# haesungpyun/seoul_tourism_recommendation_NGCF

Measured on NVIDIA B200. Metric: ngcf_epoch_time_fwd_bwd_bpr, lower is better.
Workload: dtype f32

## Files before the change

seoul_tourism_recommendation_ngcf_b200/csrc/dense.cu:

```cuda
#include <stdlib.h>
#include <string.h>

#include "common.cuh"

namespace {

__global__ void pack_weights_kernel(const float* __restrict__ W1, const float* __restrict__ b1,
                                    const float* __restrict__ W2, const float* __restrict__ b2, int d_in, int d_out,
                                    float* __restrict__ wcat, float* __restrict__ bias_eff) {
    const int total = 2 * d_in * d_out;
    for (int i = blockIdx.x * blockDim.x + threadIdx.x; i < total; i += gridDim.x * blockDim.x) {
        const int k = i / d_out, o = i % d_out;
        wcat[i] = k < d_in ? W1[o * d_in + k] : W2[o * d_in + (k - d_in)];
    }
    for (int o = blockIdx.x * blockDim.x + threadIdx.x; o < d_out; o += gridDim.x * blockDim.x)
        bias_eff[o] = 2.0f * b1[o] + b2[o];
}

struct PackAllArgs {
    const float* W1[NGCF_MAX_LAYERS];
    const float* b1[NGCF_MAX_LAYERS];
    const float* W2[NGCF_MAX_LAYERS];
    const float* b2[NGCF_MAX_LAYERS];
    float* wcat[NGCF_MAX_LAYERS];
// ... 492 lines not shown

extern "C" int ngcf_dense_bwd(const float* gE_next, const int32_t* slot, const float* gsum, int64_t ld_gsum,
                              int col_off, const float* E_out, const float* S, const float* E, int64_t n_rows,
                              int d_in, int d_out, const float* W1, const float* W2, float slope,
                              const float* mess_mult, const uint32_t* mess_bits, float mess_p, uint64_t seed,
                              const uint64_t* seed_dev, int layer, int64_t row_offset, int gh_normalized, float* gS,
                              float* gEl, float* gW1, float* gb1, float* gW2, float* gb2, float* gM_scratch, void* stream) {
    NGCF_REQUIRE(E_out && S && E && W1 && W2 && gS && gEl && gW1 && gb1 && gW2 && gb2, "dense_bwd: null pointer");
    NGCF_REQUIRE(!slot || gsum, "dense_bwd: slot given without gsum");
    NGCF_REQUIRE(d_in > 0 && d_in <= NGCF_MAX_WIDTH && d_out > 0 && d_out <= NGCF_MAX_WIDTH,
                 "dense_bwd: widths %d -> %d not in [1,%d]", d_in, d_out, NGCF_MAX_WIDTH);
    NGCF_REQUIRE(mess_p >= 0.f && mess_p < 1.f, "dense_bwd: mess_p %f not in [0,1)", mess_p);
    NGCF_REQUIRE(n_rows >= 0 && n_rows < ((int64_t)1 << 31), "dense_bwd: n_rows %lld", (long long)n_rows);
    if (n_rows == 0) return NGCF_OK;
    if (ngcf_use_tensor_cores() && gM_scratch && ngcf_dense_bwd_tc_eligible(d_in, d_out, gh_normalized) && aligned16(S) &&
        aligned16(E) && aligned16(gS) && aligned16(gEl) && aligned16(gM_scratch))
        return ngcf_dense_bwd_tc(gE_next, slot, gsum, ld_gsum, col_off, E_out, S, E, n_rows, d_in, d_out, W1, W2,
                                 slope, mess_mult, mess_bits, mess_p, seed, seed_dev, layer, row_offset, gh_normalized, gS,
                                 gEl, gW1, gb1, gW2, gb2, gM_scratch, as_stream(stream));
    BwdArgs a{gE_next, slot, gsum, ld_gsum, col_off, E_out, S, E, n_rows, d_in, d_out, W1, W2, slope, mess_mult,
              mess_bits, mess_p, seed, seed_dev, layer, gS, gEl, gW1, gb1, gW2, gb2, 0, row_offset, gh_normalized};
    int rc;
    if (d_in <= 64 && d_out <= 64) {
        constexpr int DC = 64, R = 64, T = 256;
        a.n_tiles = (int)ceil_div64(n_rows, R);
        const size_t smem = sizeof(float) * (2 * DC * DC + 3 * R * (DC + 4) + (T / 32) * DC);
        const int grid = (int)min((int64_t)a.n_tiles, (int64_t)ngcf_num_sms() * 2);
        if ((rc = set_smem(dense_bwd_kernel<DC, R, T>, smem)) != NGCF_OK) return rc;
        dense_bwd_kernel<DC, R, T><<<grid, T, smem, as_stream(stream)>>>(a);
    } else {
        constexpr int DC = 128, R = 32, T = 512;
// ... 45 lines not shown
```

seoul_tourism_recommendation_ngcf_b200/csrc/dense_tc.cu:

```cuda
#include <stdlib.h>
#include <string.h>

#include "tc.cuh"
#include "tmap.h"

namespace {

using namespace tc;

__device__ long long g_bwd_dbg[4][8][8];
__device__ int g_bwd_dbg_on = 0;
#define BWD_STAMP(role, it, k)                                                   \
    do {                                                                         \
        if (dbg && lane == 0 && (it) < 8) g_bwd_dbg[role][it][k] = clock64();    \
    } while (0)

constexpr int TC_ROWS = 128;
constexpr int TC_EPI_WARPS = 4;
constexpr int TC_LOAD_WARPS = 8;
constexpr int TC_THREADS = (TC_EPI_WARPS + 1 + TC_LOAD_WARPS) * 32;
constexpr int TC_MAX_KB = 4;
constexpr int TC_A_BLOCK = TC_ROWS * 128;

struct FwdTcArgs {
// ... 528 lines not shown
    float slope;
    const float* mess_mult;
    const uint32_t* mess_bits;
    float mess_p;
    uint64_t seed;
    const uint64_t* seed_dev;
    int layer;
    float* gS;
    float* gEl;
    float* gM;
    float* gb1;
    float* gb2;
    int n_tiles;
    int64_t row_off;
    int d_out_full, out_off, d_in_full, in_off, accumulate, first_in;
    int pf;
};

struct BwdBars {
    uint64_t full_gm, empty_gm, tmem_full[2], tmem_empty[2];
    uint32_t tmem_base;
    float colsum[64];
};

__device__ __forceinline__ uint32_t es_off(int r, int c) { return (uint32_t)r * 256u + (uint32_t)((c ^ (r & 15)) << 4); }

template <int MM, bool PRE>
__global__ void __launch_bounds__(TC_THREADS, 1) dense_bwd_tc_kernel(BwdTcArgs a) {
    extern __shared__ uint8_t smem_raw[];
    const uint32_t base = (smem_u32(smem_raw) + 1023u) & ~1023u;
    uint8_t* smem = smem_raw + (base - smem_u32(smem_raw));
    constexpr int d_in = 64;
    const int d_out = a.d_out;
    const int KBo = d_out / 32;
    uint8_t* GM_hi = smem;
    uint8_t* GM_lo = GM_hi + KBo * TC_A_BLOCK;
    uint8_t* BT_hi = GM_lo + KBo * TC_A_BLOCK;
    uint8_t* BT_lo = BT_hi + KBo * TC_A_BLOCK;
    uint8_t* E_s = BT_lo + KBo * TC_A_BLOCK;
    uint8_t* S_s = E_s + TC_ROWS * 256;
    BwdBars* bars = reinterpret_cast<BwdBars*>(S_s + TC_ROWS * 256);

    const int tid = threadIdx.x, warp = tid >> 5, lane = tid & 31;
    pdl_launch_dependents();

    if (tid == 0) {
        mbar_init(&bars->full_gm, TC_LOAD_WARPS);
        mbar_init(&bars->empty_gm, 1);
        for (int i = 0; i < 2; ++i) {
            mbar_init(&bars->tmem_full[i], 1);
            mbar_init(&bars->tmem_empty[i], TC_EPI_WARPS);
        }
        fence_mbar_init();
    }
    if (warp == TC_EPI_WARPS) tmem_alloc(&bars->tmem_base, 256);
    if (tid < 64) bars->colsum[tid] = 0.f;
    auto prefetch_tile = [&](int tile, bool fwd_tensors, bool grad) {
        const int64_t row0 = (int64_t)tile * TC_ROWS;
        if (row0 >= a.n_rows) return;
        const int64_t nr = a.n_rows - row0 < TC_ROWS ? a.n_rows - row0 : TC_ROWS;
        if (fwd_tensors) {
            l2_prefetch_bulk(a.E_out + row0 * a.d_out_full, (uint32_t)(nr * a.d_out_full * 4));
            l2_prefetch_bulk(a.S + row0 * a.d_in_full, (uint32_t)(nr * a.d_in_full * 4));
            l2_prefetch_bulk(a.E + row0 * a.d_in_full, (uint32_t)(nr * a.d_in_full * 4));
        }
        if (grad && a.gE_next) l2_prefetch_bulk(a.gE_next + row0 * a.d_out_full, (uint32_t)(nr * a.d_out_full * 4));
    };
    if (a.pf > 0 && warp == TC_EPI_WARPS + 1 && lane == 0) {
        for (int i = 0; i < a.pf; ++i) {
            const int tile = blockIdx.x + i * gridDim.x;
            if (tile < a.n_tiles) prefetch_tile(tile, true, false);
        }
    }
    for (int i = tid; i < 128 * KBo * 8; i += TC_THREADS) {
        const int n = i & 127, c = (i >> 7) & 7, kb = i >> 10;
        const float* W = (n < d_in ? a.W1 : a.W2) + a.in_off + (n & 63);
        const int o0 = a.out_off + kb * 32 + c * 4;
        const int64_t ldw = a.d_in_full;
        float4 w = make_float4(W[(int64_t)o0 * ldw], W[(int64_t)(o0 + 1) * ldw], W[(int64_t)(o0 + 2) * ldw],
                               W[(int64_t)(o0 + 3) * ldw]);
        float4 hi, lo;
        split_tf32(w, hi, lo);
        const uint32_t off = kb * TC_A_BLOCK + sw128_offset(n, c);
        *reinterpret_cast<float4*>(BT_hi + off) = hi;
        *reinterpret_cast<float4*>(BT_lo + off) = lo;
    }
    fence_proxy_async_smem();
    tc_fence_before_sync();
    __syncthreads();
    tc_fence_after_sync();
    pdl_wait();
    const uint32_t tmem_base = bars->tmem_base;
    const int n_my = (a.n_tiles - (int)blockIdx.x + (int)gridDim.x - 1) / (int)gridDim.x;
    const bool dbg = g_bwd_dbg_on == 1 && blockIdx.x == 0 && (warp == 0 || warp == TC_EPI_WARPS || warp == TC_EPI_WARPS + 1);
    if (dbg && lane == 0 && warp == 0) g_bwd_dbg[0][7][7] = clock64();

    if (warp < TC_EPI_WARPS) {
        const int r = warp * 32 + lane;
        uint8_t* e_row = E_s + r * 256;
        uint8_t* s_row = S_s + r * 256;
        const int sw = r & 15;
        const int c = lane & 15, hsel = lane >> 4;
        const uint32_t e_s32 = smem_u32(E_s), s_s32 = smem_u32(S_s);
        auto fill = [&](int tile) {
            const int64_t row0 = (int64_t)tile * TC_ROWS;
#pragma unroll 4
            for (int i = 0; i < 16; ++i) {
                const int rl = warp * 32 + 2 * i + hsel;
                const int64_t row = row0 + rl;
// ... 53 lines not shown
                    float* ps = a.gS + row * a.d_in_full + a.in_off + c * 4;
                    float* pe = a.gEl + row * a.d_in_full + a.in_off + c * 4;
                    if (a.accumulate) {
                        const float4 x0 = ld_f4(ps), y0 = ld_f4(pe);
                        x.x += x0.x; x.y += x0.y; x.z += x0.z; x.w += x0.w;
                        y.x += y0.x; y.y += y0.y; y.z += y0.z; y.w += y0.w;
                    }
                    st_f4(ps, x);
                    st_f4(pe, y);
                }
            }
            __syncwarp();
            BWD_STAMP(0, it, 4);
            if (it + 1 < n_my) fill(tile + gridDim.x);
        }
    } else if (warp == TC_EPI_WARPS) {
        const uint32_t idesc1 = umma_idesc_tf32(TC_ROWS, 2 * d_in, 0, 0);
        if (a.pf > 0 && lane == 0)
            for (int i = 0; i < a.pf && i < n_my; ++i) prefetch_tile(blockIdx.x + i * gridDim.x, false, true);
        for (int it = 0; it < n_my; ++it) {
            const int buf = it & 1;
            BWD_STAMP(1, it, 0);
            if (a.pf > 0 && lane == 0 && it + a.pf < n_my) prefetch_tile(blockIdx.x + (it + a.pf) * gridDim.x, true, true);
            mbar_wait(&bars->full_gm, it & 1);
            BWD_STAMP(1, it, 1);
            mbar_wait(&bars->tmem_empty[buf], ((it >> 1) & 1) ^ 1);
            BWD_STAMP(1, it, 2);
            tc_fence_after_sync();
            if (lane == 0) {
                const uint32_t tmem_t = tmem_base + buf * 128;
                const uint32_t gm_hi = smem_u32(GM_hi), gm_lo = smem_u32(GM_lo);
                uint32_t acc1 = 0;
                for (int kb = 0; kb < KBo; ++kb) {
#pragma unroll
                    for (int k = 0; k < 4; ++k) {
                        const uint32_t off = kb * TC_A_BLOCK + k * 32;
                        const uint64_t dah = umma_desc_sw128(gm_hi + off, 16, 1024);
                        const uint64_t dal = umma_desc_sw128(gm_lo + off, 16, 1024);
                        const uint64_t dbh = umma_desc_sw128(smem_u32(BT_hi) + off, 16, 1024);
                        const uint64_t dbl = umma_desc_sw128(smem_u32(BT_lo) + off, 16, 1024);
                        umma_tf32(tmem_t, dah, dbh, idesc1, acc1);
                        umma_tf32(tmem_t, dal, dbh, idesc1, 1);
                        umma_tf32(tmem_t, dah, dbl, idesc1, 1);
                        acc1 = 1;
                    }
                }
                umma_commit(&bars->tmem_full[buf]);
                umma_commit(&bars->empty_gm);
            }
            __syncwarp();
            BWD_STAMP(1, it, 3);
        }
    } else {
        const int lw = warp - (TC_EPI_WARPS + 1);
        const int hl = lane & 15, hsel = lane >> 4;
        const int c0 = hl * 4;
        const bool col_ok = c0 < d_out;
        const uint64_t seed = MM == MM_HASH ? ngcf_seed(a.seed, a.seed_dev) : 0ull;
        const uint32_t thr = ngcf_threshold16(a.mess_p);
        const float inv_keep = 1.0f / (1.0f - a.mess_p);
        float4 colsum = make_float4(0.f, 0.f, 0.f, 0.f);
        constexpr int HP = TC_ROWS / (4 * TC_LOAD_WARPS);
        struct Half {
            float4 e[HP], gn[HP];
            int sl[HP];
        };
        auto issue = [&](Half& h, int tile, int half) {
            const int64_t row0 = (int64_t)tile * TC_ROWS;
#pragma unroll
            for (int j = 0; j < HP; ++j) {
                const int64_t row = row0 + 2 * (lw + TC_LOAD_WARPS * (half * HP + j)) + hsel;
                const bool ok = row < a.n_rows && col_ok;
                h.e[j] = h.gn[j] = make_float4(0.f, 0.f, 0.f, 0.f);
                h.sl[j] = -1;
                if (ok) {
                    h.e[j] = ld_stream_f4(a.E_out + row * a.d_out_full + a.out_off + c0);
                    if (a.gE_next) h.gn[j] = ld_stream_f4(a.gE_next + row * a.d_out_full + a.out_off + c0);
                    if (a.slot) h.sl[j] = a.slot[row];
                }
            }
        };
        auto compute = [&](Half& h, int tile, int half) {
            const int64_t row0 = (int64_t)tile * TC_ROWS;
            if (PRE) {
#pragma unroll
                for (int j = 0; j < HP; ++j) {
                    const int s = h.sl[j];
                    if (s >= 0) {
                        const float* gp = a.gsum + (int64_t)s * a.ld_gsum + a.col_off + a.out_off + c0;
                        h.gn[j].x += gp[0]; h.gn[j].y += gp[1]; h.gn[j].z += gp[2]; h.gn[j].w += gp[3];
                    }
                }
            } else {
#pragma unroll
                for (int j = 0; j < HP; ++j) {
                    const int s = h.sl[j];
                    if (__any_sync(FULL_MASK, s >= 0)) {
                        float4 gh = make_float4(0.f, 0.f, 0.f, 0.f);
                        if (s >= 0) {
                            const float* gp = a.gsum + (int64_t)s * a.ld_gsum + a.col_off + a.out_off + c0;
                            gh = make_float4(gp[0], gp[1], gp[2], gp[3]);
                        }
                        const float4 e = h.e[j];
                        float nrm2 = e.x * e.x + e.y * e.y + e.z * e.z + e.w * e.w;
                        float dot = e.x * gh.x + e.y * gh.y + e.z * gh.z + e.w * gh.w;
#pragma unroll
                        for (int o = 8; o > 0; o >>= 1) {
                            nrm2 += __shfl_xor_sync(FULL_MASK, nrm2, o);
                            dot += __shfl_xor_sync(FULL_MASK, dot, o);
                        }
                        if (s >= 0) {
                            const float rn = 1.0f / fmaxf(sqrtf(nrm2), 1e-12f);
                            const float hd = dot * rn;
                            h.gn[j].x += (gh.x - (e.x * rn) * hd) * rn;
                            h.gn[j].y += (gh.y - (e.y * rn) * hd) * rn;
                            h.gn[j].z += (gh.z - (e.z * rn) * hd) * rn;
                            h.gn[j].w += (gh.w - (e.w * rn) * hd) * rn;
                        }
                    }
                }
            }
#pragma unroll
            for (int j = 0; j < HP; ++j) {
                const int r = 2 * (lw + TC_LOAD_WARPS * (half * HP + j)) + hsel;
                const int64_t row = row0 + r;
                const bool in = row < a.n_rows && col_ok;
                const float4 e = h.e[j];
                float4 g = h.gn[j];
                float4 mult = make_float4(1.f, 1.f, 1.f, 1.f);
                if (MM == MM_MULT) {
                    if (in) mult = ld_f4(a.mess_mult + row * a.d_out_full + a.out_off + c0);
                } else if (MM == MM_BITS) {
                    uint32_t w = 0;
                    if (in) w = a.mess_bits[row * ((a.d_out_full + 31) >> 5) + ((a.out_off + c0) >> 5)] >> ((a.out_off + c0) & 31);
                    mult = make_float4(w & 1u ? inv_keep : 0.f, w & 2u ? inv_keep : 0.f, w & 4u ? inv_keep : 0.f,
                                       w & 8u ? inv_keep : 0.f);
                } else if (MM == MM_HASH) {
                    mult = mess_multiplier4_pre(thr, inv_keep, seed, a.layer,
                                                (uint64_t)((row + a.row_off) * a.d_out_full + a.out_off + c0) >> 2);
                }
                g.x *= mult.x * (e.x > 0.f ? 1.f : a.slope);
                g.y *= mult.y * (e.y > 0.f ? 1.f : a.slope);
                g.z *= mult.z * (e.z > 0.f ? 1.f : a.slope);
                g.w *= mult.w * (e.w > 0.f ? 1.f : a.slope);
                if (!in) g = make_float4(0.f, 0.f, 0.f, 0.f);
                if (in && a.first_in) st_f4(a.gM + row * a.d_out_full + a.out_off + c0, g);
                colsum.x += g.x; colsum.y += g.y; colsum.z += g.z; colsum.w += g.w;
                if (col_ok) {
                    float4 hi, lo;
                    split_tf32_trunc(g, hi, lo);
                    const uint32_t off = (hl >> 3) * TC_A_BLOCK + sw128_offset(r, hl & 7);
                    *reinterpret_cast<float4*>(GM_hi + off) = hi;
                    *reinterpret_cast<float4*>(GM_lo + off) = lo;
                }
            }
        };
        Half h0, h1;
        if (n_my > 0) issue(h0, blockIdx.x, 0);
        for (int it = 0; it < n_my; ++it) {
            const int tile = blockIdx.x + it * gridDim.x;
            BWD_STAMP(2, it, 0);
            issue(h1, tile, 1);
            BWD_STAMP(2, it, 1);
            mbar_wait(&bars->empty_gm, (it & 1) ^ 1);
            BWD_STAMP(2, it, 2);
            compute(h0, tile, 0);
            BWD_STAMP(3, it, 0);
            if (it + 1 < n_my) issue(h0, tile + gridDim.x, 0);
            BWD_STAMP(3, it, 1);
            compute(h1, tile, 1);
            BWD_STAMP(3, it, 2);
            fence_proxy_async_smem();
            BWD_STAMP(3, it, 3);
            __syncwarp();
            if (lane == 0) mbar_arrive(&bars->full_gm);
            BWD_STAMP(2, it, 3);
        }
        colsum.x += __shfl_xor_sync(FULL_MASK, colsum.x, 16);
        colsum.y += __shfl_xor_sync(FULL_MASK, colsum.y, 16);
        colsum.z += __shfl_xor_sync(FULL_MASK, colsum.z, 16);
        colsum.w += __shfl_xor_sync(FULL_MASK, colsum.w, 16);
        if (hsel == 0 && col_ok) {
            atomicAdd(&bars->colsum[c0 + 0], colsum.x);
            atomicAdd(&bars->colsum[c0 + 1], colsum.y);
            atomicAdd(&bars->colsum[c0 + 2], colsum.z);
            atomicAdd(&bars->colsum[c0 + 3], colsum.w);
        }
        asm volatile("bar.sync 1, %0;" ::"n"(TC_LOAD_WARPS * 32) : "memory");
        const int lt = tid - (TC_EPI_WARPS + 1) * 32;
        if (lt < d_out && a.first_in) {
            const float cs = bars->colsum[lt];
            atomicAdd(a.gb2 + a.out_off + lt, cs);
            atomicAdd(a.gb1 + a.out_off + lt, 2.0f * cs);
        }
    }

    tc_fence_before_sync();
    __syncthreads();
    if (dbg && lane == 0 && warp == 0) g_bwd_dbg[1][7][7] = clock64();
    if (warp == TC_EPI_WARPS) {
        tc_fence_after_sync();
        tmem_dealloc(tmem_base, 256);
    }
}

constexpr int WG_ROWS = 64;
constexpr int WG_BLOCK = WG_ROWS * 128;

struct WgradArgs {
    const float* S;
    const float* E;
    const float* gM;
    int64_t n_rows;
    int d_out;
    float* gW1;
    float* gW2;
    int n_chunks;
// ... 275 lines not shown
bool ngcf_dense_bwd_tc_eligible(int d_in, int d_out, int gh_normalized) {
    if (d_in == 64 && (d_out == 32 || d_out == 64)) return true;
    return (d_in == 64 || d_in == 128) && (d_out == 64 || d_out == 128) && (d_out <= 64 || gh_normalized);
}

int ngcf_dense_bwd_tc(const float* gE_next, const int32_t* slot, const float* gsum, int64_t ld_gsum, int col_off,
                      const float* E_out, const float* S, const float* E, int64_t n_rows, int d_in, int d_out,
                      const float* W1, const float* W2, float slope, const float* mess_mult, const uint32_t* mess_bits,
                      float mess_p, uint64_t seed, const uint64_t* seed_dev, int layer, int64_t row_offset,
                      int gh_normalized, float* gS, float* gEl, float* gW1, float* gb1, float* gW2, float* gb2,
                      float* gM_scratch, cudaStream_t st) {
    const int bn = d_out > 64 ? 64 : d_out;
    const int IH = d_in / 64, OH = d_out / bn;
    const int KBo = bn / 32;
    const int n_tiles = (int)ceil_div64(n_rows, TC_ROWS);
    const size_t smem = 1024 + (size_t)4 * KBo * TC_A_BLOCK + 2 * TC_ROWS * 256 + sizeof(BwdBars);
    const int grid = (int)min((int64_t)n_tiles, (int64_t)ngcf_num_sms());
    void (*kern)(BwdTcArgs) = nullptr;
    const bool pre = gh_normalized != 0;
    switch (mess_mode(mess_mult, mess_bits, mess_p)) {
        case MM_NONE: kern = pre ? dense_bwd_tc_kernel<MM_NONE, true> : dense_bwd_tc_kernel<MM_NONE, false>; break;
        case MM_MULT: kern = pre ? dense_bwd_tc_kernel<MM_MULT, true> : dense_bwd_tc_kernel<MM_MULT, false>; break;
        case MM_BITS: kern = pre ? dense_bwd_tc_kernel<MM_BITS, true> : dense_bwd_tc_kernel<MM_BITS, false>; break;
        default: kern = pre ? dense_bwd_tc_kernel<MM_HASH, true> : dense_bwd_tc_kernel<MM_HASH, false>; break;
    }
    NGCF_CUDA(cudaFuncSetAttribute(kern, cudaFuncAttributeMaxDynamicSharedMemorySize, 227 * 1024));
    NGCF_CUDA(cudaFuncSetAttribute(wgrad_tc_kernel, cudaFuncAttributeMaxDynamicSharedMemorySize, 227 * 1024));
    for (int ih = 0; ih < IH; ++ih)
        for (int oh = 0; oh < OH; ++oh) {
            BwdTcArgs a{gE_next, slot, gsum, ld_gsum, col_off, E_out, S, E, n_rows, 64, bn, W1, W2, slope, mess_mult,
                        mess_bits, mess_p, seed, seed_dev, layer, gS, gEl, gM_scratch, gb1, gb2, n_tiles, row_offset};
            a.d_out_full = d_out; a.out_off = oh * bn; a.d_in_full = d_in; a.in_off = ih * 64;
            a.accumulate = oh > 0; a.first_in = ih == 0;
            const bool contiguous = d_out == bn && d_in == 64 && ((uintptr_t)E_out & 15) == 0 && ((uintptr_t)S & 15) == 0 &&
                                    ((uintptr_t)E & 15) == 0 && ((uintptr_t)gE_next & 15) == 0 && bn % 4 == 0;
            a.pf = contiguous ? dense_prefetch_tiles() : 0;
            NGCF_CUDA(ngcf_launch_pdl(kern, dim3(grid), dim3(TC_THREADS), smem, st, a));
            NGCF_LAUNCH_OK("dense_bwd_tc_kernel");
        }
    const int n_chunks = (int)ceil_div64(n_rows, WG_ROWS);
    const size_t smem2 = 1024 + (size_t)2 * (8 + 2 * KBo) * WG_BLOCK + sizeof(WgBars);
    const int grid2 = (int)min((int64_t)n_chunks, (int64_t)ngcf_num_sms());
    cudaStream_t ws = st;
    if (g_wgrad_stream && g_wgrad_stream != st) {
        static cudaEvent_t ev[64] = {};
        int dev = 0;
        NGCF_CUDA(cudaGetDevice(&dev));
        if (!ev[dev & 63]) NGCF_CUDA(cudaEventCreateWithFlags(&ev[dev & 63], cudaEventDisableTiming));
        NGCF_CUDA(cudaEventRecord(ev[dev & 63], st));
        NGCF_CUDA(cudaStreamWaitEvent(g_wgrad_stream, ev[dev & 63], 0));
        ws = g_wgrad_stream;
        g_wgrad_forked = 1;
// ... 18 lines not shown
```

seoul_tourism_recommendation_ngcf_b200/csrc/tc.cuh:

```cuda
#pragma once
#include "common.cuh"

namespace tc {

__device__ __forceinline__ uint32_t smem_u32(const void* p) { return (uint32_t)__cvta_generic_to_shared(p); }

__device__ __forceinline__ void mbar_init(uint64_t* bar, uint32_t count) {
    asm volatile("mbarrier.init.shared::cta.b64 [%0], %1;" ::"r"(smem_u32(bar)), "r"(count) : "memory");
}
__device__ __forceinline__ void fence_mbar_init() { asm volatile("fence.mbarrier_init.release.cluster;" ::: "memory"); }
__device__ __forceinline__ void mbar_arrive(uint64_t* bar) {
    asm volatile("mbarrier.arrive.shared::cta.b64 _, [%0];" ::"r"(smem_u32(bar)) : "memory");
}
__device__ __forceinline__ void mbar_wait(uint64_t* bar, uint32_t parity) {
    const uint32_t addr = smem_u32(bar);
    uint32_t done = 0;
    for (uint32_t spin = 0; ; ++spin) {
        asm volatile(
            "{\n\t.reg .pred p;\n\t"
            "mbarrier.try_wait.parity.shared::cta.b64 p, [%1], %2;\n\t"
            "selp.u32 %0, 1, 0, p;\n\t}"
            : "=r"(done)
            : "r"(addr), "r"(parity)
            : "memory");
        if (done) break;
        if (spin > (1u << 28)) __trap();
    }
}
__device__ __forceinline__ void mbar_expect_tx(uint64_t* bar, uint32_t bytes) {
    asm volatile("mbarrier.arrive.expect_tx.shared::cta.b64 _, [%0], %1;" ::"r"(smem_u32(bar)), "r"(bytes) : "memory");
}

__device__ __forceinline__ void tma_load_2d(uint32_t dst_smem, const void* tmap, int x, int y, uint64_t* bar) {
    asm volatile(
        "cp.async.bulk.tensor.2d.shared::cluster.global.tile.mbarrier::complete_tx::bytes [%0], [%1, {%2, %3}], [%4];"
        ::"r"(dst_smem), "l"(tmap), "r"(x), "r"(y), "r"(smem_u32(bar))
        : "memory");
}
__device__ __forceinline__ void tma_prefetch_desc(const void* tmap) {
    asm volatile("prefetch.tensormap [%0];" ::"l"(tmap) : "memory");
}

#ifdef NGCF_NO_PROXY_FENCE
__device__ __forceinline__ void fence_proxy_async_smem() {}
#else
__device__ __forceinline__ void fence_proxy_async_smem() { asm volatile("fence.proxy.async.shared::cta;" ::: "memory"); }
#endif

__device__ __forceinline__ void cp_async16(uint32_t dst_smem, const void* src, uint32_t src_bytes) {
    asm volatile("cp.async.cg.shared.global [%0], [%1], 16, %2;" ::"r"(dst_smem), "l"(src), "r"(src_bytes) : "memory");
}
__device__ __forceinline__ void cp_async_wait_all() { asm volatile("cp.async.wait_all;" ::: "memory"); }

// ... 25 lines not shown

__host__ __device__ constexpr uint32_t umma_idesc_tf32(int M, int N, int a_mn_major, int b_mn_major) {
    return (1u << 4) | (2u << 7) | (2u << 10) | ((uint32_t)a_mn_major << 15) | ((uint32_t)b_mn_major << 16) |
           ((uint32_t)(N >> 3) << 17) | ((uint32_t)(M >> 4) << 24);
}

__device__ __forceinline__ void umma_tf32(uint32_t tmem_d, uint64_t desc_a, uint64_t desc_b, uint32_t idesc,
                                          uint32_t accumulate) {
    asm volatile(
        "{\n\t.reg .pred p;\n\t"
        "setp.ne.b32 p, %4, 0;\n\t"
        "tcgen05.mma.cta_group::1.kind::tf32 [%0], %1, %2, %3, p;\n\t}"
        ::"r"(tmem_d), "l"(desc_a), "l"(desc_b), "r"(idesc), "r"(accumulate)
        : "memory");
}
__device__ __forceinline__ void umma_commit(uint64_t* bar) {
    asm volatile("tcgen05.commit.cta_group::1.mbarrier::arrive::one.shared::cluster.b64 [%0];" ::"r"(smem_u32(bar))
                 : "memory");
}

__device__ __forceinline__ void tmem_ld_32x32(uint32_t taddr, float (&v)[32]) {
    uint32_t r[32];
    asm volatile(
        "tcgen05.ld.sync.aligned.32x32b.x32.b32 "
        "{%0, %1, %2, %3, %4, %5, %6, %7, %8, %9, %10, %11, %12, %13, %14, %15, "
        "%16, %17, %18, %19, %20, %21, %22, %23, %24, %25, %26, %27, %28, %29, %30, %31}, [%32];"
        : "=r"(r[0]), "=r"(r[1]), "=r"(r[2]), "=r"(r[3]), "=r"(r[4]), "=r"(r[5]), "=r"(r[6]), "=r"(r[7]), "=r"(r[8]),
          "=r"(r[9]), "=r"(r[10]), "=r"(r[11]), "=r"(r[12]), "=r"(r[13]), "=r"(r[14]), "=r"(r[15]), "=r"(r[16]),
          "=r"(r[17]), "=r"(r[18]), "=r"(r[19]), "=r"(r[20]), "=r"(r[21]), "=r"(r[22]), "=r"(r[23]), "=r"(r[24]),
          "=r"(r[25]), "=r"(r[26]), "=r"(r[27]), "=r"(r[28]), "=r"(r[29]), "=r"(r[30]), "=r"(r[31])
        : "r"(taddr)
        : "memory");
    asm volatile("tcgen05.wait::ld.sync.aligned;" ::: "memory");
#pragma unroll
    for (int i = 0; i < 32; ++i) v[i] = __uint_as_float(r[i]);
}

__device__ __forceinline__ float rna_tf32(float x) {
    return __uint_as_float((__float_as_uint(x) + 0x1000u) & 0xffffe000u);
}
__device__ __forceinline__ void split_tf32(float x, float& hi, float& lo) {
    hi = rna_tf32(x);
    lo = rna_tf32(x - hi);
}
__device__ __forceinline__ void split_tf32(const float4& x, float4& hi, float4& lo) {
    split_tf32(x.x, hi.x, lo.x);
    split_tf32(x.y, hi.y, lo.y);
    split_tf32(x.z, hi.z, lo.z);
    split_tf32(x.w, hi.w, lo.w);
}

__device__ __forceinline__ void split_tf32_trunc(const float4& x, float4& hi, float4& lo) {
    hi = x;
    lo.x = x.x - __uint_as_float(__float_as_uint(x.x) & 0xffffe000u);
    lo.y = x.y - __uint_as_float(__float_as_uint(x.y) & 0xffffe000u);
    lo.z = x.z - __uint_as_float(__float_as_uint(x.z) & 0xffffe000u);
    lo.w = x.w - __uint_as_float(__float_as_uint(x.w) & 0xffffe000u);
}

__device__ __forceinline__ uint32_t sw128_offset(uint32_t r, uint32_t c) {
    return (r >> 3) * 1024u + (r & 7u) * 128u + ((c ^ (r & 7u)) << 4);
}

__device__ __forceinline__ uint32_t sw128b32_offset(uint32_t r, uint32_t c) {
    return r * 128u + ((((c >> 1) ^ (r & 3u)) << 5) | ((c & 1u) << 4));
}

}
```

Before: 0.4921.

## Feed dense backward via TMA ring and TMEM-resident A operand

Reworks the tensor-core dense backward kernel. A dedicated TMA warp now loads E_out and gE_next tiles into a 3-stage swizzled shared-memory ring and writes gM back with TMA stores. The load warps compute the hi/lo split of gM and store it into TMEM, so the MMA reads operand A from TMEM instead of shared memory, and the gM buffer is double-buffered. This replaces the old per-thread streaming loads and L2 prefetching, aiming to overlap memory traffic with compute and free shared memory. In exchange it adds barrier complexity, doubles the TMEM allocation, and requires 16-byte alignment of E_out and gE_next.

```diff
diff --git a/seoul_tourism_recommendation_ngcf_b200/csrc/dense.cu b/seoul_tourism_recommendation_ngcf_b200/csrc/dense.cu
--- a/seoul_tourism_recommendation_ngcf_b200/csrc/dense.cu
+++ b/seoul_tourism_recommendation_ngcf_b200/csrc/dense.cu
@@ -530,7 +530,8 @@
     NGCF_REQUIRE(n_rows >= 0 && n_rows < ((int64_t)1 << 31), "dense_bwd: n_rows %lld", (long long)n_rows);
     if (n_rows == 0) return NGCF_OK;
     if (ngcf_use_tensor_cores() && gM_scratch && ngcf_dense_bwd_tc_eligible(d_in, d_out, gh_normalized) && aligned16(S) &&
-        aligned16(E) && aligned16(gS) && aligned16(gEl) && aligned16(gM_scratch))
+        aligned16(E) && aligned16(gS) && aligned16(gEl) && aligned16(gM_scratch) && aligned16(E_out) &&
+        (!gE_next || aligned16(gE_next)))
         return ngcf_dense_bwd_tc(gE_next, slot, gsum, ld_gsum, col_off, E_out, S, E, n_rows, d_in, d_out, W1, W2,
                                  slope, mess_mult, mess_bits, mess_p, seed, seed_dev, layer, row_offset, gh_normalized, gS,
                                  gEl, gW1, gb1, gW2, gb2, gM_scratch, as_stream(stream));
diff --git a/seoul_tourism_recommendation_ngcf_b200/csrc/dense_tc.cu b/seoul_tourism_recommendation_ngcf_b200/csrc/dense_tc.cu
--- a/seoul_tourism_recommendation_ngcf_b200/csrc/dense_tc.cu
+++ b/seoul_tourism_recommendation_ngcf_b200/csrc/dense_tc.cu
@@ -566,11 +566,26 @@
     int n_tiles;
     int64_t row_off;
     int d_out_full, out_off, d_in_full, in_off, accumulate, first_in;
-    int pf;
 };
 
+struct BwdTmaArgs {
+    BwdTcArgs b;
+    alignas(64) CUtensorMap tmEo;
+    alignas(64) CUtensorMap tmGn;
+    alignas(64) CUtensorMap tmGm;
+};
+
+constexpr int BW_MMA_WARP = TC_EPI_WARPS;
+constexpr int BW_LOAD_WARP0 = BW_MMA_WARP + 1;
+constexpr int BW_TMA_WARP = BW_LOAD_WARP0 + TC_LOAD_WARPS;
+constexpr int BW_THREADS = (BW_TMA_WARP + 1) * 32;
+constexpr int BW_RING = 3;
+constexpr int BW_STAGE = 2 * TC_A_BLOCK;
+constexpr uint32_t BW_TM_GM = 256, BW_TM_COLS = 512;
+
 struct BwdBars {
-    uint64_t full_gm, empty_gm, tmem_full[2], tmem_empty[2];
+    uint64_t raw_full[2][2], raw_done[BW_RING];
+    uint64_t full_gm[2], empty_gm[2], tmem_full[2], tmem_empty[2];
     uint32_t tmem_base;
     float colsum[64];
 };
@@ -578,16 +593,16 @@
 __device__ __forceinline__ uint32_t es_off(int r, int c) { return (uint32_t)r * 256u + (uint32_t)((c ^ (r & 15)) << 4); }
 
 template <int MM, bool PRE>
-__global__ void __launch_bounds__(TC_THREADS, 1) dense_bwd_tc_kernel(BwdTcArgs a) {
+__global__ void __launch_bounds__(BW_THREADS, 1) dense_bwd_tc_kernel(const __grid_constant__ BwdTmaArgs p) {
     extern __shared__ uint8_t smem_raw[];
+    const BwdTcArgs& a = p.b;
     const uint32_t base = (smem_u32(smem_raw) + 1023u) & ~1023u;
     uint8_t* smem = smem_raw + (base - smem_u32(smem_raw));
     constexpr int d_in = 64;
     const int d_out = a.d_out;
     const int KBo = d_out / 32;
-    uint8_t* GM_hi = smem;
-    uint8_t* GM_lo = GM_hi + KBo * TC_A_BLOCK;
-    uint8_t* BT_hi = GM_lo + KBo * TC_A_BLOCK;
+    uint8_t* RAW = smem;
+    uint8_t* BT_hi = RAW + BW_RING * BW_STAGE;
     uint8_t* BT_lo = BT_hi + KBo * TC_A_BLOCK;
     uint8_t* E_s = BT_lo + KBo * TC_A_BLOCK;
     uint8_t* S_s = E_s + TC_ROWS * 256;
@@ -597,34 +612,22 @@
     pdl_launch_dependents();
 
     if (tid == 0) {
-        mbar_init(&bars->full_gm, TC_LOAD_WARPS);
-        mbar_init(&bars->empty_gm, 1);
+        for (int i = 0; i < 4; ++i) mbar_init(&bars->raw_full[i >> 1][i & 1], 1);
+        for (int i = 0; i < BW_RING; ++i) mbar_init(&bars->raw_done[i], 4);
         for (int i = 0; i < 2; ++i) {
+            mbar_init(&bars->full_gm[i], 4 * KBo);
+            mbar_init(&bars->empty_gm[i], 1);
             mbar_init(&bars->tmem_full[i], 1);
             mbar_init(&bars->tmem_empty[i], TC_EPI_WARPS);
         }
         fence_mbar_init();
-    }
-    if (warp == TC_EPI_WARPS) tmem_alloc(&bars->tmem_base, 256);
+        tma_prefetch_desc(&p.tmEo);
+        tma_prefetch_desc(&p.tmGn);
+        tma_prefetch_desc(&p.tmGm);
+    }
+    if (warp == BW_MMA_WARP) tmem_alloc(&bars->tmem_base, BW_TM_COLS);
     if (tid < 64) bars->colsum[tid] = 0.f;
-    auto prefetch_tile = [&](int tile, bool fwd_tensors, bool grad) {
-        const int64_t row0 = (int64_t)tile * TC_ROWS;
-        if (row0 >= a.n_rows) return;
-        const int64_t nr = a.n_rows - row0 < TC_ROWS ? a.n_rows - row0 : TC_ROWS;
-        if (fwd_tensors) {
-            l2_prefetch_bulk(a.E_out + row0 * a.d_out_full, (uint32_t)(nr * a.d_out_full * 4));
-            l2_prefetch_bulk(a.S + row0 * a.d_in_full, (uint32_t)(nr * a.d_in_full * 4));
-            l2_prefetch_bulk(a.E + row0 * a.d_in_full, (uint32_t)(nr * a.d_in_full * 4));
-        }
-        if (grad && a.gE_next) l2_prefetch_bulk(a.gE_next + row0 * a.d_out_full, (uint32_t)(nr * a.d_out_full * 4));
-    };
-    if (a.pf > 0 && warp == TC_EPI_WARPS + 1 && lane == 0) {
-        for (int i = 0; i < a.pf; ++i) {
-            const int tile = blockIdx.x + i * gridDim.x;
-            if (tile < a.n_tiles) prefetch_tile(tile, true, false);
-        }
-    }
-    for (int i = tid; i < 128 * KBo * 8; i += TC_THREADS) {
+    for (int i = tid; i < 128 * KBo * 8; i += BW_THREADS) {
         const int n = i & 127, c = (i >> 7) & 7, kb = i >> 10;
         const float* W = (n < d_in ? a.W1 : a.W2) + a.in_off + (n & 63);
         const int o0 = a.out_off + kb * 32 + c * 4;
@@ -644,7 +647,8 @@
     pdl_wait();
     const uint32_t tmem_base = bars->tmem_base;
     const int n_my = (a.n_tiles - (int)blockIdx.x + (int)gridDim.x - 1) / (int)gridDim.x;
-    const bool dbg = g_bwd_dbg_on == 1 && blockIdx.x == 0 && (warp == 0 || warp == TC_EPI_WARPS || warp == TC_EPI_WARPS + 1);
+    const bool dbg = g_bwd_dbg_on == 1 && blockIdx.x == 0 &&
+                     (warp == 0 || warp == BW_MMA_WARP || warp == BW_LOAD_WARP0 || warp == BW_TMA_WARP);
     if (dbg && lane == 0 && warp == 0) g_bwd_dbg[0][7][7] = clock64();
 
     if (warp < TC_EPI_WARPS) {
@@ -728,193 +732,221 @@
             BWD_STAMP(0, it, 4);
             if (it + 1 < n_my) fill(tile + gridDim.x);
         }
-    } else if (warp == TC_EPI_WARPS) {
+    } else if (warp == BW_MMA_WARP) {
         const uint32_t idesc1 = umma_idesc_tf32(TC_ROWS, 2 * d_in, 0, 0);
-        if (a.pf > 0 && lane == 0)
-            for (int i = 0; i < a.pf && i < n_my; ++i) prefetch_tile(blockIdx.x + i * gridDim.x, false, true);
         for (int it = 0; it < n_my; ++it) {
             const int buf = it & 1;
             BWD_STAMP(1, it, 0);
-            if (a.pf > 0 && lane == 0 && it + a.pf < n_my) prefetch_tile(blockIdx.x + (it + a.pf) * gridDim.x, true, true);
-            mbar_wait(&bars->full_gm, it & 1);
+            mbar_wait(&bars->full_gm[buf], (it >> 1) & 1);
             BWD_STAMP(1, it, 1);
             mbar_wait(&bars->tmem_empty[buf], ((it >> 1) & 1) ^ 1);
             BWD_STAMP(1, it, 2);
             tc_fence_after_sync();
             if (lane == 0) {
                 const uint32_t tmem_t = tmem_base + buf * 128;
-                const uint32_t gm_hi = smem_u32(GM_hi), gm_lo = smem_u32(GM_lo);
+                const uint32_t gm_hi = tmem_base + BW_TM_GM + buf * 128, gm_lo = gm_hi + 64;
                 uint32_t acc1 = 0;
                 for (int kb = 0; kb < KBo; ++kb) {
 #pragma unroll
                     for (int k = 0; k < 4; ++k) {
                         const uint32_t off = kb * TC_A_BLOCK + k * 32;
-                        const uint64_t dah = umma_desc_sw128(gm_hi + off, 16, 1024);
-                        const uint64_t dal = umma_desc_sw128(gm_lo + off, 16, 1024);
+                        const uint32_t col = kb * 32 + k * 8;
                         const uint64_t dbh = umma_desc_sw128(smem_u32(BT_hi) + off, 16, 1024);
                         const uint64_t dbl = umma_desc_sw128(smem_u32(BT_lo) + off, 16, 1024);
-                        umma_tf32(tmem_t, dah, dbh, idesc1, acc1);
-                        umma_tf32(tmem_t, dal, dbh, idesc1, 1);
-                        umma_tf32(tmem_t, dah, dbl, idesc1, 1);
+                        umma_tf32_ta(tmem_t, gm_hi + col, dbh, idesc1, acc1);
+                        umma_tf32_ta(tmem_t, gm_lo + col, dbh, idesc1, 1);
+                        umma_tf32_ta(tmem_t, gm_hi + col, dbl, idesc1, 1);
                         acc1 = 1;
                     }
                 }
                 umma_commit(&bars->tmem_full[buf]);
-                umma_commit(&bars->empty_gm);
+                umma_commit(&bars->empty_gm[buf]);
             }
             __syncwarp();
             BWD_STAMP(1, it, 3);
         }
+    } else if (warp == BW_TMA_WARP) {
+        if (lane == 0) {
+            const int n_q = n_my * KBo;
+            const uint32_t tx = a.gE_next ? BW_STAGE : TC_A_BLOCK;
+            for (int q = 0; q < n_q + BW_RING; ++q) {
+                const int s = q % BW_RING;
+                if (q >= BW_RING) {
+                    const int qd = q - BW_RING;
+                    mbar_wait(&bars->raw_done[s], (qd / BW_RING) & 1);
+                    BWD_STAMP(3, qd / KBo, (qd % KBo) * 3 + 0);
+                    if (a.first_in) {
+                        const int tile = blockIdx.x + (qd / KBo) * gridDim.x;
+                        tma_store_2d(&p.tmGm, a.out_off + (qd % KBo) * 32, tile * TC_ROWS, smem_u32(RAW + s * BW_STAGE));
+                        tma_store_commit();
+                        tma_store_wait_read();
+                    }
+                    BWD_STAMP(3, qd / KBo, (qd % KBo) * 3 + 1);
+                }
+                if (q < n_q) {
+                    const int it = q / KBo, h = q % KBo;
+                    const int tile = blockIdx.x + it * gridDim.x, x = a.out_off + h * 32;
+                    const uint32_t dst = smem_u32(RAW + s * BW_STAGE);
+                    uint64_t* full = &bars->raw_full[h][it & 1];
+                    mbar_expect_tx(full, tx);
+                    tma_load_2d(dst, &p.tmEo, x, tile * TC_ROWS, full);
+                    if (a.gE_next) tma_load_2d(dst + TC_A_BLOCK, &p.tmGn, x, tile * TC_ROWS, full);
+                    BWD_STAMP(3, q / KBo, (q % KBo) * 3 + 2);
+                }
+            }
+            tma_store_wait_all();
+        }
     } else {
-        const int lw = warp - (TC_EPI_WARPS + 1);
-        const int hl = lane & 15, hsel = lane >> 4;
-        const int c0 = hl * 4;
-        const bool col_ok = c0 < d_out;
+        const int lw = warp - BW_LOAD_WARP0;
+        const int h = lw >> 2;
+        const int r = (warp & 3) * 32 + lane;
+        const int gc0 = a.out_off + h * 32;
         const uint64_t seed = MM == MM_HASH ? ngcf_seed(a.seed, a.seed_dev) : 0ull;
         const uint32_t thr = ngcf_threshold16(a.mess_p);
         const float inv_keep = 1.0f / (1.0f - a.mess_p);
-        float4 colsum = make_float4(0.f, 0.f, 0.f, 0.f);
-        constexpr int HP = TC_ROWS / (4 * TC_LOAD_WARPS);
-        struct Half {
-            float4 e[HP], gn[HP];
-            int sl[HP];
-        };
-        auto issue = [&](Half& h, int tile, int half) {
-            const int64_t row0 = (int64_t)tile * TC_ROWS;
-#pragma unroll
-            for (int j = 0; j < HP; ++j) {
-                const int64_t row = row0 + 2 * (lw + TC_LOAD_WARPS * (half * HP + j)) + hsel;
-                const bool ok = row < a.n_rows && col_ok;
-                h.e[j] = h.gn[j] = make_float4(0.f, 0.f, 0.f, 0.f);
-                h.sl[j] = -1;
-                if (ok) {
-                    h.e[j] = ld_stream_f4(a.E_out + row * a.d_out_full + a.out_off + c0);
-                    if (a.gE_next) h.gn[j] = ld_stream_f4(a.gE_next + row * a.d_out_full + a.out_off + c0);
-                    if (a.slot) h.sl[j] = a.slot[row];
-                }
-            }
-        };
-        auto compute = [&](Half& h, int tile, int half) {
-            const int64_t row0 = (int64_t)tile * TC_ROWS;
-            if (PRE) {
-#pragma unroll
-                for (int j = 0; j < HP; ++j) {
-                    const int s = h.sl[j];
-                    if (s >= 0) {
-                        const float* gp = a.gsum + (int64_t)s * a.ld_gsum + a.col_off + a.out_off + c0;
-                        h.gn[j].x += gp[0]; h.gn[j].y += gp[1]; h.gn[j].z += gp[2]; h.gn[j].w += gp[3];
+        float cs[32];
+#pragma unroll
+        for (int j = 0; j < 32; ++j) cs[j] = 0.f;
+        if (h < KBo) {
+            auto slot_of = [&](int it) -> int {
+                const int64_t row = (int64_t)(blockIdx.x + it * gridDim.x) * TC_ROWS + r;
+                return it < n_my && a.slot && row < a.n_rows ? a.slot[row] : -1;
+            };
+            int sl_next = slot_of(0);
+            for (int it = 0; it < n_my; ++it) {
+                const int tile = blockIdx.x + it * gridDim.x;
+                const int buf = it & 1, q = it * KBo + h, s = q % BW_RING;
+                const int64_t row = (int64_t)tile * TC_ROWS + r;
+                const bool in = row < a.n_rows;
+                const int sl = sl_next;
+                sl_next = slot_of(it + 1);
+                float gh[32];
+                const float* gp = a.gsum + (int64_t)(sl >= 0 ? sl : 0) * a.ld_gsum + a.col_off + a.out_off;
+#pragma unroll
+                for (int j = 0; j < 32; ++j) gh[j] = sl >= 0 ? gp[h * 32 + j] : 0.f;
+                BWD_STAMP(2, it, 0);
+                mbar_wait(&bars->raw_full[h][it & 1], (it >> 1) & 1);
+                BWD_STAMP(2, it, 1);
+                mbar_wait(&bars->empty_gm[buf], ((it >> 1) & 1) ^ 1);
+                tc_fence_after_sync();
+                BWD_STAMP(2, it, 2);
+                uint8_t* eo = RAW + s * BW_STAGE + r * 128;
+                const uint8_t* gn = eo + TC_A_BLOCK;
+                float rn = 0.f, hd = 0.f;
+                if (!PRE && sl >= 0) {
+                    auto part = [&](int hj, int c, float& pn, float& pd) {
+                        float4 e = make_float4(0.f, 0.f, 0.f, 0.f), g = e;
+                        if (hj == h) {
+                            e = *reinterpret_cast<const float4*>(eo + ((c ^ (r & 7)) << 4));
+                            g = make_float4(gh[4 * c], gh[4 * c + 1], gh[4 * c + 2], gh[4 * c + 3]);
+                        } else if (hj < KBo) {
+                            e = ld_f4(a.E_out + row * a.d_out_full + hj * 32 + 4 * c);
+                            const float* go = gp + hj * 32 + 4 * c;
+                            g = make_float4(go[0], go[1], go[2], go[3]);
+                        }
+                        pn = e.x * e.x + e.y * e.y + e.z * e.z + e.w * e.w;
+                        pd = e.x * g.x + e.y * g.y + e.z * g.z + e.w * g.w;
+                    };
+                    float pn[8], pd[8];
+#pragma unroll
+                    for (int c = 0; c < 8; ++c) {
+                        float n0, d0, n1, d1;
+                        part(0, c, n0, d0);
+                        part(1, c, n1, d1);
+                        pn[c] = n0 + n1;
+                        pd[c] = d0 + d1;
                     }
-                }
-            } else {
-#pragma unroll
-                for (int j = 0; j < HP; ++j) {
-                    const int s = h.sl[j];
-                    if (__any_sync(FULL_MASK, s >= 0)) {
-                        float4 gh = make_float4(0.f, 0.f, 0.f, 0.f);
-                        if (s >= 0) {
-                            const float* gp = a.gsum + (int64_t)s * a.ld_gsum + a.col_off + a.out_off + c0;
-                            gh = make_float4(gp[0], gp[1], gp[2], gp[3]);
+#pragma unroll
+                    for (int o = 4; o > 0; o >>= 1)
+#pragma unroll
+                        for (int j = 0; j < o; ++j) {
+                            pn[j] += pn[j + o];
+                            pd[j] += pd[j + o];
                         }
-                        const float4 e = h.e[j];
-                        float nrm2 = e.x * e.x + e.y * e.y + e.z * e.z + e.w * e.w;
-                        float dot = e.x * gh.x + e.y * gh.y + e.z * gh.z + e.w * gh.w;
-#pragma unroll
-                        for (int o = 8; o > 0; o >>= 1) {
-                            nrm2 += __shfl_xor_sync(FULL_MASK, nrm2, o);
-                            dot += __shfl_xor_sync(FULL_MASK, dot, o);
+                    rn = 1.0f / fmaxf(sqrtf(pn[0]), 1e-12f);
+                    hd = pd[0] * rn;
+                }
+                uint32_t wbits = 0;
+                if (MM == MM_BITS && in) wbits = a.mess_bits[row * ((a.d_out_full + 31) >> 5) + (gc0 >> 5)];
+                const uint32_t t_hi = tmem_base + ((uint32_t)((warp & 3) * 32) << 16) + BW_TM_GM + buf * 128 + h * 32;
+#pragma unroll
+                for (int c2 = 0; c2 < 4; ++c2) {
+                    float vhi[8], vlo[8];
+#pragma unroll
+                    for (int cc = 0; cc < 2; ++cc) {
+                        const int c = c2 * 2 + cc;
+                        const uint32_t off = (uint32_t)((c ^ (r & 7)) << 4);
+                        const float4 e = *reinterpret_cast<const float4*>(eo + off);
+                        float4 g = a.gE_next ? *reinterpret_cast<const float4*>(gn + off) : make_float4(0.f, 0.f, 0.f, 0.f);
+                        if (PRE && sl >= 0) {
+                            g.x += gh[4 * c]; g.y += gh[4 * c + 1]; g.z += gh[4 * c + 2]; g.w += gh[4 * c + 3];
+                        } else if (sl >= 0) {
+                            g.x += (gh[4 * c] - (e.x * rn) * hd) * rn;
+                            g.y += (gh[4 * c + 1] - (e.y * rn) * hd) * rn;
+                            g.z += (gh[4 * c + 2] - (e.z * rn) * hd) * rn;
+                            g.w += (gh[4 * c + 3] - (e.w * rn) * hd) * rn;
                         }
-                        if (s >= 0) {
-                            const float rn = 1.0f / fmaxf(sqrtf(nrm2), 1e-12f);
-                            const float hd = dot * rn;
-                            h.gn[j].x += (gh.x - (e.x * rn) * hd) * rn;
-                            h.gn[j].y += (gh.y - (e.y * rn) * hd) * rn;
-                            h.gn[j].z += (gh.z - (e.z * rn) * hd) * rn;
-                            h.gn[j].w += (gh.w - (e.w * rn) * hd) * rn;
+                        float4 mult = make_float4(1.f, 1.f, 1.f, 1.f);
+                        if (MM == MM_MULT) {
+                            if (in) mult = ld_f4(a.mess_mult + row * a.d_out_full + gc0 + 4 * c);
+                        } else if (MM == MM_BITS) {
+                            const uint32_t w = wbits >> (4 * c);
+                            mult = make_float4(w & 1u ? inv_keep : 0.f, w & 2u ? inv_keep : 0.f, w & 4u ? inv_keep : 0.f,
+                                               w & 8u ? inv_keep : 0.f);
+                        } else if (MM == MM_HASH) {
+                            mult = mess_multiplier4_pre(thr, inv_keep, seed, a.layer,
+                                                        (uint64_t)((row + a.row_off) * a.d_out_full + gc0 + 4 * c) >> 2);
+                        }
+                        g.x *= mult.x * (e.x > 0.f ? 1.f : a.slope);
+                        g.y *= mult.y * (e.y > 0.f ? 1.f : a.slope);
+                        g.z *= mult.z * (e.z > 0.f ? 1.f : a.slope);
+                        g.w *= mult.w * (e.w > 0.f ? 1.f : a.slope);
+                        if (!in) g = make_float4(0.f, 0.f, 0.f, 0.f);
+                        *reinterpret_cast<float4*>(eo + off) = g;
+                        cs[4 * c] += g.x; cs[4 * c + 1] += g.y; cs[4 * c + 2] += g.z; cs[4 * c + 3] += g.w;
+                        const float gv[4] = {g.x, g.y, g.z, g.w};
+#pragma unroll
+                        for (int k = 0; k < 4; ++k) {
+                            vhi[cc * 4 + k] = trunc_tf32(gv[k]);
+                            vlo[cc * 4 + k] = trunc_tf32(gv[k] - vhi[cc * 4 + k]);
                         }
                     }
-                }
-            }
-#pragma unroll
-            for (int j = 0; j < HP; ++j) {
-                const int r = 2 * (lw + TC_LOAD_WARPS * (half * HP + j)) + hsel;
-                const int64_t row = row0 + r;
-                const bool in = row < a.n_rows && col_ok;
-                const float4 e = h.e[j];
-                float4 g = h.gn[j];
-                float4 mult = make_float4(1.f, 1.f, 1.f, 1.f);
-                if (MM == MM_MULT) {
-                    if (in) mult = ld_f4(a.mess_mult + row * a.d_out_full + a.out_off + c0);
-                } else if (MM == MM_BITS) {
-                    uint32_t w = 0;
-                    if (in) w = a.mess_bits[row * ((a.d_out_full + 31) >> 5) + ((a.out_off + c0) >> 5)] >> ((a.out_off + c0) & 31);
-                    mult = make_float4(w & 1u ? inv_keep : 0.f, w & 2u ? inv_keep : 0.f, w & 4u ? inv_keep : 0.f,
-                                       w & 8u ? inv_keep : 0.f);
-                } else if (MM == MM_HASH) {
-                    mult = mess_multiplier4_pre(thr, inv_keep, seed, a.layer,
-                                                (uint64_t)((row + a.row_off) * a.d_out_full + a.out_off + c0) >> 2);
-                }
-                g.x *= mult.x * (e.x > 0.f ? 1.f : a.slope);
-                g.y *= mult.y * (e.y > 0.f ? 1.f : a.slope);
-                g.z *= mult.z * (e.z > 0.f ? 1.f : a.slope);
-                g.w *= mult.w * (e.w > 0.f ? 1.f : a.slope);
-                if (!in) g = make_float4(0.f, 0.f, 0.f, 0.f);
-                if (in && a.first_in) st_f4(a.gM + row * a.d_out_full + a.out_off + c0, g);
-                colsum.x += g.x; colsum.y += g.y; colsum.z += g.z; colsum.w += g.w;
-                if (col_ok) {
-                    float4 hi, lo;
-                    split_tf32_trunc(g, hi, lo);
-                    const uint32_t off = (hl >> 3) * TC_A_BLOCK + sw128_offset(r, hl & 7);
-                    *reinterpret_cast<float4*>(GM_hi + off) = hi;
-                    *reinterpret_cast<float4*>(GM_lo + off) = lo;
-                }
-            }
-        };
-        Half h0, h1;
-        if (n_my > 0) issue(h0, blockIdx.x, 0);
-        for (int it = 0; it < n_my; ++it) {
-            const int tile = blockIdx.x + it * gridDim.x;
-            BWD_STAMP(2, it, 0);
-            issue(h1, tile, 1);
-            BWD_STAMP(2, it, 1);
-            mbar_wait(&bars->empty_gm, (it & 1) ^ 1);
-            BWD_STAMP(2, it, 2);
-            compute(h0, tile, 0);
-            BWD_STAMP(3, it, 0);
-            if (it + 1 < n_my) issue(h0, tile + gridDim.x, 0);
-            BWD_STAMP(3, it, 1);
-            compute(h1, tile, 1);
-            BWD_STAMP(3, it, 2);
-            fence_proxy_async_smem();
-            BWD_STAMP(3, it, 3);
-            __syncwarp();
-            if (lane == 0) mbar_arrive(&bars->full_gm);
-            BWD_STAMP(2, it, 3);
-        }
-        colsum.x += __shfl_xor_sync(FULL_MASK, colsum.x, 16);
-        colsum.y += __shfl_xor_sync(FULL_MASK, colsum.y, 16);
-        colsum.z += __shfl_xor_sync(FULL_MASK, colsum.z, 16);
-        colsum.w += __shfl_xor_sync(FULL_MASK, colsum.w, 16);
-        if (hsel == 0 && col_ok) {
-            atomicAdd(&bars->colsum[c0 + 0], colsum.x);
-            atomicAdd(&bars->colsum[c0 + 1], colsum.y);
-            atomicAdd(&bars->colsum[c0 + 2], colsum.z);
-            atomicAdd(&bars->colsum[c0 + 3], colsum.w);
-        }
+                    tmem_st_32x32_x8(t_hi + c2 * 8, vhi);
+                    tmem_st_32x32_x8(t_hi + 64 + c2 * 8, vlo);
+                }
+                tmem_st_wait();
+                fence_proxy_async_smem();
+                tc_fence_before_sync();
+                __syncwarp();
+                if (lane == 0) {
+                    mbar_arrive(&bars->raw_done[s]);
+                    mbar_arrive(&bars->full_gm[buf]);
+                }
+                BWD_STAMP(2, it, 3);
+            }
+        }
+        float mine = 0.f;
+#pragma unroll
+        for (int j = 0; j < 32; ++j) {
+            const float v = warp_sum(cs[j]);
+            if (lane == j) mine = v;
+        }
+        if (h < KBo) atomicAdd(&bars->colsum[h * 32 + lane], mine);
         asm volatile("bar.sync 1, %0;" ::"n"(TC_LOAD_WARPS * 32) : "memory");
-        const int lt = tid - (TC_EPI_WARPS + 1) * 32;
+        const int lt = tid - BW_LOAD_WARP0 * 32;
         if (lt < d_out && a.first_in) {
-            const float cs = bars->colsum[lt];
-            atomicAdd(a.gb2 + a.out_off + lt, cs);
-            atomicAdd(a.gb1 + a.out_off + lt, 2.0f * cs);
+            const float v = bars->colsum[lt];
+            atomicAdd(a.gb2 + a.out_off + lt, v);
+            atomicAdd(a.gb1 + a.out_off + lt, 2.0f * v);
         }
     }
 
     tc_fence_before_sync();
     __syncthreads();
     if (dbg && lane == 0 && warp == 0) g_bwd_dbg[1][7][7] = clock64();
-    if (warp == TC_EPI_WARPS) {
+    if (warp == BW_MMA_WARP) {
         tc_fence_after_sync();
-        tmem_dealloc(tmem_base, 256);
+        tmem_dealloc(tmem_base, BW_TM_COLS);
     }
 }
 
@@ -1220,9 +1252,10 @@
     const int IH = d_in / 64, OH = d_out / bn;
     const int KBo = bn / 32;
     const int n_tiles = (int)ceil_div64(n_rows, TC_ROWS);
-    const size_t smem = 1024 + (size_t)4 * KBo * TC_A_BLOCK + 2 * TC_ROWS * 256 + sizeof(BwdBars);
+    const size_t smem = 1024 + (size_t)BW_RING * BW_STAGE + (size_t)2 * KBo * TC_A_BLOCK + 2 * TC_ROWS * 256 +
+                        sizeof(BwdBars);
     const int grid = (int)min((int64_t)n_tiles, (int64_t)ngcf_num_sms());
-    void (*kern)(BwdTcArgs) = nullptr;
+    void (*kern)(const BwdTmaArgs) = nullptr;
     const bool pre = gh_normalized != 0;
     switch (mess_mode(mess_mult, mess_bits, mess_p)) {
         case MM_NONE: kern = pre ? dense_bwd_tc_kernel<MM_NONE, true> : dense_bwd_tc_kernel<MM_NONE, false>; break;
@@ -1232,16 +1265,24 @@
     }
     NGCF_CUDA(cudaFuncSetAttribute(kern, cudaFuncAttributeMaxDynamicSharedMemorySize, 227 * 1024));
     NGCF_CUDA(cudaFuncSetAttribute(wgrad_tc_kernel, cudaFuncAttributeMaxDynamicSharedMemorySize, 227 * 1024));
+    BwdTmaArgs p{};
+    int rc = ngcf_encode_tmap_2d(&p.tmEo, E_out, (uint64_t)n_rows, (uint64_t)d_out, (uint64_t)d_out, 32, TC_ROWS,
+                                 CU_TENSOR_MAP_SWIZZLE_128B);
+    if (rc == 0)
+        rc = ngcf_encode_tmap_2d(&p.tmGn, gE_next ? gE_next : E_out, (uint64_t)n_rows, (uint64_t)d_out, (uint64_t)d_out,
+                                 32, TC_ROWS, CU_TENSOR_MAP_SWIZZLE_128B);
+    if (rc == 0)
+        rc = ngcf_encode_tmap_2d(&p.tmGm, gM_scratch, (uint64_t)n_rows, (uint64_t)d_out, (uint64_t)d_out, 32, TC_ROWS,
+                                 CU_TENSOR_MAP_SWIZZLE_128B);
+    NGCF_REQUIRE(rc == 0, "dense_bwd: cuTensorMapEncodeTiled failed (%d)", rc);
     for (int ih = 0; ih < IH; ++ih)
         for (int oh = 0; oh < OH; ++oh) {
             BwdTcArgs a{gE_next, slot, gsum, ld_gsum, col_off, E_out, S, E, n_rows, 64, bn, W1, W2, slope, mess_mult,
                         mess_bits, mess_p, seed, seed_dev, layer, gS, gEl, gM_scratch, gb1, gb2, n_tiles, row_offset};
             a.d_out_full = d_out; a.out_off = oh * bn; a.d_in_full = d_in; a.in_off = ih * 64;
             a.accumulate = oh > 0; a.first_in = ih == 0;
-            const bool contiguous = d_out == bn && d_in == 64 && ((uintptr_t)E_out & 15) == 0 && ((uintptr_t)S & 15) == 0 &&
-                                    ((uintptr_t)E & 15) == 0 && ((uintptr_t)gE_next & 15) == 0 && bn % 4 == 0;
-            a.pf = contiguous ? dense_prefetch_tiles() : 0;
-            NGCF_CUDA(ngcf_launch_pdl(kern, dim3(grid), dim3(TC_THREADS), smem, st, a));
+            p.b = a;
+            NGCF_CUDA(ngcf_launch_pdl(kern, dim3(grid), dim3(BW_THREADS), smem, st, p));
             NGCF_LAUNCH_OK("dense_bwd_tc_kernel");
         }
     const int n_chunks = (int)ceil_div64(n_rows, WG_ROWS);
diff --git a/seoul_tourism_recommendation_ngcf_b200/csrc/tc.cuh b/seoul_tourism_recommendation_ngcf_b200/csrc/tc.cuh
--- a/seoul_tourism_recommendation_ngcf_b200/csrc/tc.cuh
+++ b/seoul_tourism_recommendation_ngcf_b200/csrc/tc.cuh
@@ -37,6 +37,14 @@
         ::"r"(dst_smem), "l"(tmap), "r"(x), "r"(y), "r"(smem_u32(bar))
         : "memory");
 }
+__device__ __forceinline__ void tma_store_2d(const void* tmap, int x, int y, uint32_t src_smem) {
+    asm volatile("cp.async.bulk.tensor.2d.global.shared::cta.tile.bulk_group [%0, {%1, %2}], [%3];"
+                 ::"l"(tmap), "r"(x), "r"(y), "r"(src_smem)
+                 : "memory");
+}
+__device__ __forceinline__ void tma_store_commit() { asm volatile("cp.async.bulk.commit_group;" ::: "memory"); }
+__device__ __forceinline__ void tma_store_wait_read() { asm volatile("cp.async.bulk.wait_group.read 0;" ::: "memory"); }
+__device__ __forceinline__ void tma_store_wait_all() { asm volatile("cp.async.bulk.wait_group 0;" ::: "memory"); }
 __device__ __forceinline__ void tma_prefetch_desc(const void* tmap) {
     asm volatile("prefetch.tensormap [%0];" ::"l"(tmap) : "memory");
 }
@@ -92,6 +100,15 @@
         ::"r"(tmem_d), "l"(desc_a), "l"(desc_b), "r"(idesc), "r"(accumulate)
         : "memory");
 }
+__device__ __forceinline__ void umma_tf32_ta(uint32_t tmem_d, uint32_t tmem_a, uint64_t desc_b, uint32_t idesc,
+                                             uint32_t accumulate) {
+    asm volatile(
+        "{\n\t.reg .pred p;\n\t"
+        "setp.ne.b32 p, %4, 0;\n\t"
+        "tcgen05.mma.cta_group::1.kind::tf32 [%0], [%1], %2, %3, p;\n\t}"
+        ::"r"(tmem_d), "r"(tmem_a), "l"(desc_b), "r"(idesc), "r"(accumulate)
+        : "memory");
+}
 __device__ __forceinline__ void umma_commit(uint64_t* bar) {
     asm volatile("tcgen05.commit.cta_group::1.mbarrier::arrive::one.shared::cluster.b64 [%0];" ::"r"(smem_u32(bar))
                  : "memory");
@@ -113,6 +130,15 @@
 #pragma unroll
     for (int i = 0; i < 32; ++i) v[i] = __uint_as_float(r[i]);
 }
+
+__device__ __forceinline__ void tmem_st_32x32_x8(uint32_t taddr, const float (&v)[8]) {
+    asm volatile("tcgen05.st.sync.aligned.32x32b.x8.b32 [%0], {%1, %2, %3, %4, %5, %6, %7, %8};"
+                 ::"r"(taddr), "r"(__float_as_uint(v[0])), "r"(__float_as_uint(v[1])), "r"(__float_as_uint(v[2])),
+                   "r"(__float_as_uint(v[3])), "r"(__float_as_uint(v[4])), "r"(__float_as_uint(v[5])),
+                   "r"(__float_as_uint(v[6])), "r"(__float_as_uint(v[7]))
+                 : "memory");
+}
+__device__ __forceinline__ void tmem_st_wait() { asm volatile("tcgen05.wait::st.sync.aligned;" ::: "memory"); }
 
 __device__ __forceinline__ float rna_tf32(float x) {
     return __uint_as_float((__float_as_uint(x) + 0x1000u) & 0xffffe000u);
@@ -136,6 +162,8 @@
     lo.w = x.w - __uint_as_float(__float_as_uint(x.w) & 0xffffe000u);
 }
 
+__device__ __forceinline__ float trunc_tf32(float x) { return __uint_as_float(__float_as_uint(x) & 0xffffe000u); }
+
 __device__ __forceinline__ uint32_t sw128_offset(uint32_t r, uint32_t c) {
     return (r >> 3) * 1024u + (r & 7u) * 128u + ((c ^ (r & 7u)) << 4);
 }
```

Result: faster. 0.4761, median of 6 (-3.3%).
